# distributed-lab/era-boojum

Measured on AMD Instinct MI355X. Metric: LDE+Merkle commit Goldilocks elems/s (2^22x256, LDE x4), higher is better.
Workload: dtype u64 (Goldilocks); 1 GPU; C3: 2^22 rows x 256 cols, LDE x4, Poseidon2 cap 16; rows=4194304, cols=256, lde=4, cap=16, tree_hasher=poseidon2, parallelism=single, launch=stream

## Files before the change

### era-boojum_amd/csrc/gl_asm.hpp

```cpp
#pragma once
#include <stdint.h>

namespace glasm {

__device__ __forceinline__ void mul_x1(uint32_t a00, uint32_t a10, uint32_t b00, uint32_t b10, uint32_t& z00, uint32_t& z10) {
    uint64_t q40, q42, q44, q64;
    asm volatile(
        "v_mad_u64_u32 v[2:3], %[q64], %[a10], %[b00], 0\n"
        "v_mad_u64_u32 v[0:1], %[q64], %[a00], %[b00], 0\n"
        "v_mad_u64_u32 v[4:5], %[q44], %[a00], %[b10], v[2:3]\n"
        "v_mad_u64_u32 v[6:7], %[q64], %[a10], %[b10], 0\n"
        "v_add_co_u32 v1, %[q40], v1, v4\n"
        "v_addc_co_u32 v7, %[q64], v7, 0, %[q44]\n"
        "s_nop 0\n"
        "v_addc_co_u32 v5, %[q42], v5, v6, %[q40]\n"
        "s_nop 1\n"
        "v_subb_co_u32 v0, %[q40], v0, v7, %[q42]\n"
        "s_nop 1\n"
        "v_subb_co_u32 v1, %[q40], v1, 0, %[q40]\n"
        "s_nop 1\n"
        "v_subb_co_u32 v5, %[q40], v5, 0, %[q40]\n"
        "v_mad_u64_u32 v[2:3], %[q42], v5, -1, v[0:1]\n"
        "s_nop 1\n"
        "v_cndmask_b32_e64 v8, 0, -1, %[q42]\n"
// ... 72 lines not shown
        "v_addc_co_u32 v25, %[q54], v25, v26, %[q52]\n"
        "v_subb_co_u32 v0, %[q40], v0, v7, %[q42]\n"
        "v_subb_co_u32 v10, %[q46], v10, v17, %[q48]\n"
        "v_subb_co_u32 v20, %[q52], v20, v27, %[q54]\n"
        "v_subb_co_u32 v1, %[q40], v1, 0, %[q40]\n"
        "v_subb_co_u32 v11, %[q46], v11, 0, %[q46]\n"
        "v_subb_co_u32 v21, %[q52], v21, 0, %[q52]\n"
        "v_subb_co_u32 v5, %[q40], v5, 0, %[q40]\n"
        "v_subb_co_u32 v15, %[q46], v15, 0, %[q46]\n"
        "v_subb_co_u32 v25, %[q52], v25, 0, %[q52]\n"
        "v_mad_u64_u32 v[2:3], %[q42], v5, -1, v[0:1]\n"
        "v_mad_u64_u32 v[12:13], %[q48], v15, -1, v[10:11]\n"
        "v_mad_u64_u32 v[22:23], %[q54], v25, -1, v[20:21]\n"
        "v_cndmask_b32_e64 v8, 0, -1, %[q42]\n"
        "v_cndmask_b32_e64 v18, 0, -1, %[q48]\n"
        "v_cndmask_b32_e64 v28, 0, -1, %[q54]\n"
        "v_addc_co_u32 %[z00], %[q42], v2, v8, %[q40]\n"
        "v_addc_co_u32 %[z01], %[q48], v12, v18, %[q46]\n"
        "v_addc_co_u32 %[z02], %[q54], v22, v28, %[q52]\n"
        "v_addc_co_u32 %[z10], %[q64], v3, 0, %[q42]\n"
        "v_addc_co_u32 %[z11], %[q64], v13, 0, %[q48]\n"
        "v_addc_co_u32 %[z12], %[q64], v23, 0, %[q54]\n"
        : [z00] "=&v"(z00), [z10] "=&v"(z10), [z01] "=&v"(z01), [z11] "=&v"(z11), [z02] "=&v"(z02), [z12] "=&v"(z12), [q40] "=&s"(q40), [q42] "=&s"(q42), [q44] "=&s"(q44), [q46] "=&s"(q46), [q48] "=&s"(q48), [q50] "=&s"(q50), [q52] "=&s"(q52), [q54] "=&s"(q54), [q56] "=&s"(q56), [q64] "=&s"(q64)
        : [a00] "v"(a00), [a10] "v"(a10), [b00] "v"(b00), [b10] "v"(b10), [a01] "v"(a01), [a11] "v"(a11), [b01] "v"(b01), [b11] "v"(b11), [a02] "v"(a02), [a12] "v"(a12), [b02] "v"(b02), [b12] "v"(b12)
        : "v0", "v1", "v2", "v3", "v4", "v5", "v6", "v7", "v8", "v9", "v10", "v11", "v12", "v13", "v14", "v15", "v16", "v17", "v18", "v19", "v20", "v21", "v22", "v23", "v24", "v25", "v26", "v27", "v28", "v29");
}

__device__ __forceinline__ void mul_x4(uint32_t a00, uint32_t a10, uint32_t b00, uint32_t b10, uint32_t& z00, uint32_t& z10, uint32_t a01, uint32_t a11, uint32_t b01, uint32_t b11, uint32_t& z01, uint32_t& z11, uint32_t a02, uint32_t a12, uint32_t b02, uint32_t b12, uint32_t& z02, uint32_t& z12, uint32_t a03, uint32_t a13, uint32_t b03, uint32_t b13, uint32_t& z03, uint32_t& z13) {
    uint64_t q40, q42, q44, q46, q48, q50, q52, q54, q56, q58, q60, q62, q64;
    asm volatile(
        "v_mad_u64_u32 v[2:3], %[q64], %[a10], %[b00], 0\n"
        "v_mad_u64_u32 v[12:13], %[q64], %[a11], %[b01], 0\n"
        "v_mad_u64_u32 v[22:23], %[q64], %[a12], %[b02], 0\n"
        "v_mad_u64_u32 v[32:33], %[q64], %[a13], %[b03], 0\n"
        "v_mad_u64_u32 v[0:1], %[q64], %[a00], %[b00], 0\n"
        "v_mad_u64_u32 v[10:11], %[q64], %[a01], %[b01], 0\n"
        "v_mad_u64_u32 v[20:21], %[q64], %[a02], %[b02], 0\n"
        "v_mad_u64_u32 v[30:31], %[q64], %[a03], %[b03], 0\n"
        "v_mad_u64_u32 v[4:5], %[q44], %[a00], %[b10], v[2:3]\n"
        "v_mad_u64_u32 v[14:15], %[q50], %[a01], %[b11], v[12:13]\n"
        "v_mad_u64_u32 v[24:25], %[q56], %[a02], %[b12], v[22:23]\n"
        "v_mad_u64_u32 v[34:35], %[q62], %[a03], %[b13], v[32:33]\n"
        "v_mad_u64_u32 v[6:7], %[q64], %[a10], %[b10], 0\n"
        "v_mad_u64_u32 v[16:17], %[q64], %[a11], %[b11], 0\n"
        "v_mad_u64_u32 v[26:27], %[q64], %[a12], %[b12], 0\n"
        "v_mad_u64_u32 v[36:37], %[q64], %[a13], %[b13], 0\n"
        "v_add_co_u32 v1, %[q40], v1, v4\n"
        "v_add_co_u32 v11, %[q46], v11, v14\n"
        "v_add_co_u32 v21, %[q52], v21, v24\n"
        "v_add_co_u32 v31, %[q58], v31, v34\n"
        "v_addc_co_u32 v7, %[q64], v7, 0, %[q44]\n"
        "v_addc_co_u32 v17, %[q64], v17, 0, %[q50]\n"
        "v_addc_co_u32 v27, %[q64], v27, 0, %[q56]\n"
        "v_addc_co_u32 v37, %[q64], v37, 0, %[q62]\n"
        "v_addc_co_u32 v5, %[q42], v5, v6, %[q40]\n"
        "v_addc_co_u32 v15, %[q48], v15, v16, %[q46]\n"
        "v_addc_co_u32 v25, %[q54], v25, v26, %[q52]\n"
        "v_addc_co_u32 v35, %[q60], v35, v36, %[q58]\n"
        "v_subb_co_u32 v0, %[q40], v0, v7, %[q42]\n"
        "v_subb_co_u32 v10, %[q46], v10, v17, %[q48]\n"
        "v_subb_co_u32 v20, %[q52], v20, v27, %[q54]\n"
        "v_subb_co_u32 v30, %[q58], v30, v37, %[q60]\n"
        "v_subb_co_u32 v1, %[q40], v1, 0, %[q40]\n"
        "v_subb_co_u32 v11, %[q46], v11, 0, %[q46]\n"
        "v_subb_co_u32 v21, %[q52], v21, 0, %[q52]\n"
        "v_subb_co_u32 v31, %[q58], v31, 0, %[q58]\n"
        "v_subb_co_u32 v5, %[q40], v5, 0, %[q40]\n"
        "v_subb_co_u32 v15, %[q46], v15, 0, %[q46]\n"
        "v_subb_co_u32 v25, %[q52], v25, 0, %[q52]\n"
        "v_subb_co_u32 v35, %[q58], v35, 0, %[q58]\n"
        "v_mad_u64_u32 v[2:3], %[q42], v5, -1, v[0:1]\n"
        "v_mad_u64_u32 v[12:13], %[q48], v15, -1, v[10:11]\n"
        "v_mad_u64_u32 v[22:23], %[q54], v25, -1, v[20:21]\n"
        "v_mad_u64_u32 v[32:33], %[q60], v35, -1, v[30:31]\n"
        "v_cndmask_b32_e64 v8, 0, -1, %[q42]\n"
        "v_cndmask_b32_e64 v18, 0, -1, %[q48]\n"
        "v_cndmask_b32_e64 v28, 0, -1, %[q54]\n"
        "v_cndmask_b32_e64 v38, 0, -1, %[q60]\n"
        "v_addc_co_u32 %[z00], %[q42], v2, v8, %[q40]\n"
        "v_addc_co_u32 %[z01], %[q48], v12, v18, %[q46]\n"
        "v_addc_co_u32 %[z02], %[q54], v22, v28, %[q52]\n"
        "v_addc_co_u32 %[z03], %[q60], v32, v38, %[q58]\n"
        "v_addc_co_u32 %[z10], %[q64], v3, 0, %[q42]\n"
        "v_addc_co_u32 %[z11], %[q64], v13, 0, %[q48]\n"
        "v_addc_co_u32 %[z12], %[q64], v23, 0, %[q54]\n"
        "v_addc_co_u32 %[z13], %[q64], v33, 0, %[q60]\n"
        : [z00] "=&v"(z00), [z10] "=&v"(z10), [z01] "=&v"(z01), [z11] "=&v"(z11), [z02] "=&v"(z02), [z12] "=&v"(z12), [z03] "=&v"(z03), [z13] "=&v"(z13), [q40] "=&s"(q40), [q42] "=&s"(q42), [q44] "=&s"(q44), [q46] "=&s"(q46), [q48] "=&s"(q48), [q50] "=&s"(q50), [q52] "=&s"(q52), [q54] "=&s"(q54), [q56] "=&s"(q56), [q58] "=&s"(q58), [q60] "=&s"(q60), [q62] "=&s"(q62), [q64] "=&s"(q64)
        : [a00] "v"(a00), [a10] "v"(a10), [b00] "v"(b00), [b10] "v"(b10), [a01] "v"(a01), [a11] "v"(a11), [b01] "v"(b01), [b11] "v"(b11), [a02] "v"(a02), [a12] "v"(a12), [b02] "v"(b02), [b12] "v"(b12), [a03] "v"(a03), [a13] "v"(a13), [b03] "v"(b03), [b13] "v"(b13)
        : "v0", "v1", "v2", "v3", "v4", "v5", "v6", "v7", "v8", "v9", "v10", "v11", "v12", "v13", "v14", "v15", "v16", "v17", "v18", "v19", "v20", "v21", "v22", "v23", "v24", "v25", "v26", "v27", "v28", "v29", "v30", "v31", "v32", "v33", "v34", "v35", "v36", "v37", "v38", "v39");
}

__device__ __forceinline__ void mul_sb_x4(uint32_t a00, uint32_t a10, uint32_t b00, uint32_t b10, uint32_t& z00, uint32_t& z10, uint32_t a01, uint32_t a11, uint32_t b01, uint32_t b11, uint32_t& z01, uint32_t& z11, uint32_t a02, uint32_t a12, uint32_t b02, uint32_t b12, uint32_t& z02, uint32_t& z12, uint32_t a03, uint32_t a13, uint32_t b03, uint32_t b13, uint32_t& z03, uint32_t& z13) {
    uint64_t q40, q42, q44, q46, q48, q50, q52, q54, q56, q58, q60, q62, q64;
    asm volatile(
        "v_mad_u64_u32 v[2:3], %[q64], %[a10], %[b00], 0\n"
        "v_mad_u64_u32 v[12:13], %[q64], %[a11], %[b01], 0\n"
        "v_mad_u64_u32 v[22:23], %[q64], %[a12], %[b02], 0\n"
        "v_mad_u64_u32 v[32:33], %[q64], %[a13], %[b03], 0\n"
        "v_mad_u64_u32 v[0:1], %[q64], %[a00], %[b00], 0\n"
        "v_mad_u64_u32 v[10:11], %[q64], %[a01], %[b01], 0\n"
        "v_mad_u64_u32 v[20:21], %[q64], %[a02], %[b02], 0\n"
        "v_mad_u64_u32 v[30:31], %[q64], %[a03], %[b03], 0\n"
        "v_mad_u64_u32 v[4:5], %[q44], %[a00], %[b10], v[2:3]\n"
        "v_mad_u64_u32 v[14:15], %[q50], %[a01], %[b11], v[12:13]\n"
        "v_mad_u64_u32 v[24:25], %[q56], %[a02], %[b12], v[22:23]\n"
        "v_mad_u64_u32 v[34:35], %[q62], %[a03], %[b13], v[32:33]\n"
        "v_mad_u64_u32 v[6:7], %[q64], %[a10], %[b10], 0\n"
        "v_mad_u64_u32 v[16:17], %[q64], %[a11], %[b11], 0\n"
        "v_mad_u64_u32 v[26:27], %[q64], %[a12], %[b12], 0\n"
        "v_mad_u64_u32 v[36:37], %[q64], %[a13], %[b13], 0\n"
        "v_add_co_u32 v1, %[q40], v1, v4\n"
        "v_add_co_u32 v11, %[q46], v11, v14\n"
        "v_add_co_u32 v21, %[q52], v21, v24\n"
        "v_add_co_u32 v31, %[q58], v31, v34\n"
        "v_addc_co_u32 v7, %[q64], v7, 0, %[q44]\n"
        "v_addc_co_u32 v17, %[q64], v17, 0, %[q50]\n"
        "v_addc_co_u32 v27, %[q64], v27, 0, %[q56]\n"
        "v_addc_co_u32 v37, %[q64], v37, 0, %[q62]\n"
        "v_addc_co_u32 v5, %[q42], v5, v6, %[q40]\n"
        "v_addc_co_u32 v15, %[q48], v15, v16, %[q46]\n"
        "v_addc_co_u32 v25, %[q54], v25, v26, %[q52]\n"
        "v_addc_co_u32 v35, %[q60], v35, v36, %[q58]\n"
        "v_subb_co_u32 v0, %[q40], v0, v7, %[q42]\n"
        "v_subb_co_u32 v10, %[q46], v10, v17, %[q48]\n"
        "v_subb_co_u32 v20, %[q52], v20, v27, %[q54]\n"
        "v_subb_co_u32 v30, %[q58], v30, v37, %[q60]\n"
        "v_subb_co_u32 v1, %[q40], v1, 0, %[q40]\n"
        "v_subb_co_u32 v11, %[q46], v11, 0, %[q46]\n"
        "v_subb_co_u32 v21, %[q52], v21, 0, %[q52]\n"
        "v_subb_co_u32 v31, %[q58], v31, 0, %[q58]\n"
        "v_subb_co_u32 v5, %[q40], v5, 0, %[q40]\n"
        "v_subb_co_u32 v15, %[q46], v15, 0, %[q46]\n"
        "v_subb_co_u32 v25, %[q52], v25, 0, %[q52]\n"
        "v_subb_co_u32 v35, %[q58], v35, 0, %[q58]\n"
        "v_mad_u64_u32 v[2:3], %[q42], v5, -1, v[0:1]\n"
        "v_mad_u64_u32 v[12:13], %[q48], v15, -1, v[10:11]\n"
        "v_mad_u64_u32 v[22:23], %[q54], v25, -1, v[20:21]\n"
        "v_mad_u64_u32 v[32:33], %[q60], v35, -1, v[30:31]\n"
        "v_cndmask_b32_e64 v8, 0, -1, %[q42]\n"
        "v_cndmask_b32_e64 v18, 0, -1, %[q48]\n"
        "v_cndmask_b32_e64 v28, 0, -1, %[q54]\n"
        "v_cndmask_b32_e64 v38, 0, -1, %[q60]\n"
        "v_addc_co_u32 %[z00], %[q42], v2, v8, %[q40]\n"
        "v_addc_co_u32 %[z01], %[q48], v12, v18, %[q46]\n"
        "v_addc_co_u32 %[z02], %[q54], v22, v28, %[q52]\n"
        "v_addc_co_u32 %[z03], %[q60], v32, v38, %[q58]\n"
        "v_addc_co_u32 %[z10], %[q64], v3, 0, %[q42]\n"
        "v_addc_co_u32 %[z11], %[q64], v13, 0, %[q48]\n"
        "v_addc_co_u32 %[z12], %[q64], v23, 0, %[q54]\n"
        "v_addc_co_u32 %[z13], %[q64], v33, 0, %[q60]\n"
        : [z00] "=&v"(z00), [z10] "=&v"(z10), [z01] "=&v"(z01), [z11] "=&v"(z11), [z02] "=&v"(z02), [z12] "=&v"(z12), [z03] "=&v"(z03), [z13] "=&v"(z13), [q40] "=&s"(q40), [q42] "=&s"(q42), [q44] "=&s"(q44), [q46] "=&s"(q46), [q48] "=&s"(q48), [q50] "=&s"(q50), [q52] "=&s"(q52), [q54] "=&s"(q54), [q56] "=&s"(q56), [q58] "=&s"(q58), [q60] "=&s"(q60), [q62] "=&s"(q62), [q64] "=&s"(q64)
        : [a00] "v"(a00), [a10] "v"(a10), [b00] "s"(b00), [b10] "s"(b10), [a01] "v"(a01), [a11] "v"(a11), [b01] "s"(b01), [b11] "s"(b11), [a02] "v"(a02), [a12] "v"(a12), [b02] "s"(b02), [b12] "s"(b12), [a03] "v"(a03), [a13] "v"(a13), [b03] "s"(b03), [b13] "s"(b13)
        : "v0", "v1", "v2", "v3", "v4", "v5", "v6", "v7", "v8", "v9", "v10", "v11", "v12", "v13", "v14", "v15", "v16", "v17", "v18", "v19", "v20", "v21", "v22", "v23", "v24", "v25", "v26", "v27", "v28", "v29", "v30", "v31", "v32", "v33", "v34", "v35", "v36", "v37", "v38", "v39");
}

__device__ __forceinline__ void reduce_x1(uint64_t L0, uint32_t Hlo0, uint32_t Hhi0, uint64_t& z0) {
    uint64_t q40, q64;
    asm volatile(
        "v_mad_u64_u32 v[0:1], %[q64], %[Hhi0], -1, %[L0]\n"
        "v_add_co_u32 v1, %[q40], v1, %[Hlo0]\n"
        "s_nop 1\n"
        "v_cndmask_b32_e64 v2, 0, -1, %[q40]\n"
        "v_mad_u64_u32 %[z0], %[q64], v2, 1, v[0:1]\n"
        : [z0] "=&v"(z0), [q40] "=&s"(q40), [q64] "=&s"(q64)
        : [L0] "v"(L0), [Hlo0] "v"(Hlo0), [Hhi0] "v"(Hhi0)
        : "v0", "v1", "v2", "v3");
}

__device__ __forceinline__ void reduce_x2(uint64_t L0, uint32_t Hlo0, uint32_t Hhi0, uint64_t& z0, uint64_t L1, uint32_t Hlo1, uint32_t Hhi1, uint64_t& z1) {
    uint64_t q40, q44, q64;
    asm volatile(
        "v_mad_u64_u32 v[0:1], %[q64], %[Hhi0], -1, %[L0]\n"
        "v_mad_u64_u32 v[4:5], %[q64], %[Hhi1], -1, %[L1]\n"
        "v_add_co_u32 v1, %[q40], v1, %[Hlo0]\n"
        "v_add_co_u32 v5, %[q44], v5, %[Hlo1]\n"
        "s_nop 0\n"
        "v_cndmask_b32_e64 v2, 0, -1, %[q40]\n"
        "v_cndmask_b32_e64 v6, 0, -1, %[q44]\n"
        "v_mad_u64_u32 %[z0], %[q64], v2, 1, v[0:1]\n"
        "v_mad_u64_u32 %[z1], %[q64], v6, 1, v[4:5]\n"
        : [z0] "=&v"(z0), [z1] "=&v"(z1), [q40] "=&s"(q40), [q44] "=&s"(q44), [q64] "=&s"(q64)
        : [L0] "v"(L0), [Hlo0] "v"(Hlo0), [Hhi0] "v"(Hhi0), [L1] "v"(L1), [Hlo1] "v"(Hlo1), [Hhi1] "v"(Hhi1)
        : "v0", "v1", "v2", "v3", "v4", "v5", "v6", "v7");
}

__device__ __forceinline__ void reduce_x3(uint64_t L0, uint32_t Hlo0, uint32_t Hhi0, uint64_t& z0, uint64_t L1, uint32_t Hlo1, uint32_t Hhi1, uint64_t& z1, uint64_t L2, uint32_t Hlo2, uint32_t Hhi2, uint64_t& z2) {
    uint64_t q40, q44, q48, q64;
    asm volatile(
        "v_mad_u64_u32 v[0:1], %[q64], %[Hhi0], -1, %[L0]\n"
        "v_mad_u64_u32 v[4:5], %[q64], %[Hhi1], -1, %[L1]\n"
        "v_mad_u64_u32 v[8:9], %[q64], %[Hhi2], -1, %[L2]\n"
        "v_add_co_u32 v1, %[q40], v1, %[Hlo0]\n"
        "v_add_co_u32 v5, %[q44], v5, %[Hlo1]\n"
        "v_add_co_u32 v9, %[q48], v9, %[Hlo2]\n"
        "v_cndmask_b32_e64 v2, 0, -1, %[q40]\n"
        "v_cndmask_b32_e64 v6, 0, -1, %[q44]\n"
        "v_cndmask_b32_e64 v10, 0, -1, %[q48]\n"
        "v_mad_u64_u32 %[z0], %[q64], v2, 1, v[0:1]\n"
        "v_mad_u64_u32 %[z1], %[q64], v6, 1, v[4:5]\n"
        "v_mad_u64_u32 %[z2], %[q64], v10, 1, v[8:9]\n"
        : [z0] "=&v"(z0), [z1] "=&v"(z1), [z2] "=&v"(z2), [q40] "=&s"(q40), [q44] "=&s"(q44), [q48] "=&s"(q48), [q64] "=&s"(q64)
        : [L0] "v"(L0), [Hlo0] "v"(Hlo0), [Hhi0] "v"(Hhi0), [L1] "v"(L1), [Hlo1] "v"(Hlo1), [Hhi1] "v"(Hhi1), [L2] "v"(L2), [Hlo2] "v"(Hlo2), [Hhi2] "v"(Hhi2)
        : "v0", "v1", "v2", "v3", "v4", "v5", "v6", "v7", "v8", "v9", "v10", "v11");
}

__device__ __forceinline__ void reduce_x4(uint64_t L0, uint32_t Hlo0, uint32_t Hhi0, uint64_t& z0, uint64_t L1, uint32_t Hlo1, uint32_t Hhi1, uint64_t& z1, uint64_t L2, uint32_t Hlo2, uint32_t Hhi2, uint64_t& z2, uint64_t L3, uint32_t Hlo3, uint32_t Hhi3, uint64_t& z3) {
    uint64_t q40, q44, q48, q52, q64;
    asm volatile(
        "v_mad_u64_u32 v[0:1], %[q64], %[Hhi0], -1, %[L0]\n"
        "v_mad_u64_u32 v[4:5], %[q64], %[Hhi1], -1, %[L1]\n"
        "v_mad_u64_u32 v[8:9], %[q64], %[Hhi2], -1, %[L2]\n"
        "v_mad_u64_u32 v[12:13], %[q64], %[Hhi3], -1, %[L3]\n"
        "v_add_co_u32 v1, %[q40], v1, %[Hlo0]\n"
        "v_add_co_u32 v5, %[q44], v5, %[Hlo1]\n"
        "v_add_co_u32 v9, %[q48], v9, %[Hlo2]\n"
        "v_add_co_u32 v13, %[q52], v13, %[Hlo3]\n"
        "v_cndmask_b32_e64 v2, 0, -1, %[q40]\n"
        "v_cndmask_b32_e64 v6, 0, -1, %[q44]\n"
        "v_cndmask_b32_e64 v10, 0, -1, %[q48]\n"
        "v_cndmask_b32_e64 v14, 0, -1, %[q52]\n"
        "v_mad_u64_u32 %[z0], %[q64], v2, 1, v[0:1]\n"
        "v_mad_u64_u32 %[z1], %[q64], v6, 1, v[4:5]\n"
        "v_mad_u64_u32 %[z2], %[q64], v10, 1, v[8:9]\n"
        "v_mad_u64_u32 %[z3], %[q64], v14, 1, v[12:13]\n"
        : [z0] "=&v"(z0), [z1] "=&v"(z1), [z2] "=&v"(z2), [z3] "=&v"(z3), [q40] "=&s"(q40), [q44] "=&s"(q44), [q48] "=&s"(q48), [q52] "=&s"(q52), [q64] "=&s"(q64)
        : [L0] "v"(L0), [Hlo0] "v"(Hlo0), [Hhi0] "v"(Hhi0), [L1] "v"(L1), [Hlo1] "v"(Hlo1), [Hhi1] "v"(Hhi1), [L2] "v"(L2), [Hlo2] "v"(Hlo2), [Hhi2] "v"(Hhi2), [L3] "v"(L3), [Hlo3] "v"(Hlo3), [Hhi3] "v"(Hhi3)
        : "v0", "v1", "v2", "v3", "v4", "v5", "v6", "v7", "v8", "v9", "v10", "v11", "v12", "v13", "v14", "v15");
}

__device__ __forceinline__ void add_x1(uint32_t a00, uint32_t a10, uint32_t b00, uint32_t b10, uint32_t& z00, uint32_t& z10) {
    uint64_t q40;
    asm volatile(
        "v_add_co_u32 %[z00], %[q40], %[a00], %[b00]\n"
        "s_nop 1\n"
        "v_addc_co_u32 %[z10], %[q40], %[a10], %[b10], %[q40]\n"
        "s_nop 1\n"
        "v_cndmask_b32_e64 v0, 0, -1, %[q40]\n"
        "v_add_co_u32 %[z00], %[q40], %[z00], v0\n"
        "s_nop 1\n"
        "v_addc_co_u32 %[z10], %[q40], %[z10], 0, %[q40]\n"
        "s_nop 1\n"
        "v_cndmask_b32_e64 v0, 0, -1, %[q40]\n"
        "v_add_co_u32 %[z00], %[q40], %[z00], v0\n"
        "s_nop 1\n"
        "v_addc_co_u32 %[z10], %[q40], %[z10], 0, %[q40]\n"
        : [z00] "=&v"(z00), [z10] "=&v"(z10), [q40] "=&s"(q40)
        : [a00] "v"(a00), [a10] "v"(a10), [b00] "v"(b00), [b10] "v"(b10)
        : "v0", "v1");
}

__device__ __forceinline__ void sub_x1(uint32_t a00, uint32_t a10, uint32_t b00, uint32_t b10, uint32_t& z00, uint32_t& z10) {
    uint64_t q40;
    asm volatile(
        "v_sub_co_u32 %[z00], %[q40], %[a00], %[b00]\n"
        "s_nop 1\n"
        "v_subb_co_u32 %[z10], %[q40], %[a10], %[b10], %[q40]\n"
        "s_nop 1\n"
        "v_cndmask_b32_e64 v0, 0, -1, %[q40]\n"
        "v_sub_co_u32 %[z00], %[q40], %[z00], v0\n"
        "s_nop 1\n"
        "v_subb_co_u32 %[z10], %[q40], %[z10], 0, %[q40]\n"
        "s_nop 1\n"
        "v_cndmask_b32_e64 v0, 0, -1, %[q40]\n"
        "v_sub_co_u32 %[z00], %[q40], %[z00], v0\n"
        "s_nop 1\n"
        "v_subb_co_u32 %[z10], %[q40], %[z10], 0, %[q40]\n"
        : [z00] "=&v"(z00), [z10] "=&v"(z10), [q40] "=&s"(q40)
        : [a00] "v"(a00), [a10] "v"(a10), [b00] "v"(b00), [b10] "v"(b10)
        : "v0", "v1");
}

__device__ __forceinline__ void add_x2(uint32_t a00, uint32_t a10, uint32_t b00, uint32_t b10, uint32_t& z00, uint32_t& z10, uint32_t a01, uint32_t a11, uint32_t b01, uint32_t b11, uint32_t& z01, uint32_t& z11) {
    uint64_t q40, q44;
    asm volatile(
        "v_add_co_u32 %[z00], %[q40], %[a00], %[b00]\n"
        "v_add_co_u32 %[z01], %[q44], %[a01], %[b01]\n"
        "s_nop 0\n"
        "v_addc_co_u32 %[z10], %[q40], %[a10], %[b10], %[q40]\n"
        "v_addc_co_u32 %[z11], %[q44], %[a11], %[b11], %[q44]\n"
        "s_nop 0\n"
        "v_cndmask_b32_e64 v0, 0, -1, %[q40]\n"
        "v_cndmask_b32_e64 v2, 0, -1, %[q44]\n"
        "v_add_co_u32 %[z00], %[q40], %[z00], v0\n"
        "v_add_co_u32 %[z01], %[q44], %[z01], v2\n"
        "s_nop 0\n"
        "v_addc_co_u32 %[z10], %[q40], %[z10], 0, %[q40]\n"
        "v_addc_co_u32 %[z11], %[q44], %[z11], 0, %[q44]\n"
        "s_nop 0\n"
        "v_cndmask_b32_e64 v0, 0, -1, %[q40]\n"
        "v_cndmask_b32_e64 v2, 0, -1, %[q44]\n"
        "v_add_co_u32 %[z00], %[q40], %[z00], v0\n"
        "v_add_co_u32 %[z01], %[q44], %[z01], v2\n"
        "s_nop 0\n"
        "v_addc_co_u32 %[z10], %[q40], %[z10], 0, %[q40]\n"
        "v_addc_co_u32 %[z11], %[q44], %[z11], 0, %[q44]\n"
        : [z00] "=&v"(z00), [z10] "=&v"(z10), [z01] "=&v"(z01), [z11] "=&v"(z11), [q40] "=&s"(q40), [q44] "=&s"(q44)
        : [a00] "v"(a00), [a10] "v"(a10), [b00] "v"(b00), [b10] "v"(b10), [a01] "v"(a01), [a11] "v"(a11), [b01] "v"(b01), [b11] "v"(b11)
        : "v0", "v1", "v2", "v3");
}

__device__ __forceinline__ void sub_x2(uint32_t a00, uint32_t a10, uint32_t b00, uint32_t b10, uint32_t& z00, uint32_t& z10, uint32_t a01, uint32_t a11, uint32_t b01, uint32_t b11, uint32_t& z01, uint32_t& z11) {
    uint64_t q40, q44;
    asm volatile(
        "v_sub_co_u32 %[z00], %[q40], %[a00], %[b00]\n"
        "v_sub_co_u32 %[z01], %[q44], %[a01], %[b01]\n"
        "s_nop 0\n"
// ... 791 lines not shown
```

### era-boojum_amd/csrc/poseidon2.hpp

```cpp
#pragma once
#include "gl.hpp"
#include "gl_asm.hpp"

namespace p2 {

struct RcLimbs {
    uint64_t lo[30][12];
    uint64_t hi[30][12];
};

constexpr uint64_t RC_FLAT[30][12] = {
#include "poseidon2_rc.inc"
};

constexpr RcLimbs make_rc_limbs() {
    RcLimbs r{};
    for (int i = 0; i < 30; i++)
        for (int j = 0; j < 12; j++) {
            r.lo[i][j] = RC_FLAT[i][j] & 0xFFFFFFFFull;
            r.hi[i][j] = RC_FLAT[i][j] >> 32;
        }
    return r;
}

__device__ __constant__ static const RcLimbs RCL = make_rc_limbs();

namespace sched {
constexpr uint64_t P = 0xFFFFFFFF00000001ull;
constexpr uint64_t addm(uint64_t a, uint64_t b) { return (uint64_t)(((unsigned __int128)a + b) % P); }
constexpr uint64_t subm(uint64_t a, uint64_t b) { return addm(a, P - b % P); }
constexpr uint64_t mulm(uint64_t a, uint64_t b) { return (uint64_t)(((unsigned __int128)a * b) % P); }
constexpr int SH[12] = {4, 14, 11, 8, 0, 5, 2, 9, 13, 6, 3, 12};
constexpr uint64_t FULL_RC_BOUND = ~0ull - (1ull << 41) + 1;
constexpr uint64_t LIMB_RC_BOUND = (1ull << 63) + (1ull << 62);
struct Values {
    uint64_t k[11];
    uint64_t d[10];
    uint64_t rc26[12];
};
constexpr Values derive() {
    Values v{};
    uint64_t f[12] = {RC_FLAT[4][0]};
    for (int q = 0; q < 11; q++) {
        const int r = 4 + 2 * q;
        uint64_t s = 0;
        for (int i = 1; i < 12; i++) s = addm(s, f[i]);
        v.k[q] = subm(RC_FLAT[r + 1][0], s);
        f[0] = 0;
        for (int i = 0; i < 12; i++) f[i] = addm(addm(mulm(f[i], 1ull << SH[i]), s), v.k[q]);
        s = 0;
        for (int i = 1; i < 12; i++) s = addm(s, f[i]);
        f[0] = 0;
        for (int i = 0; i < 12; i++) f[i] = addm(mulm(f[i], 1ull << SH[i]), s);
        if (q < 10) {
            v.d[q] = subm(RC_FLAT[r + 2][0], f[0]);
            f[0] = RC_FLAT[r + 2][0];
        }
    }
    for (int i = 0; i < 12; i++) v.rc26[i] = subm(RC_FLAT[26][i], f[i]);
    return v;
}
constexpr Values V = derive();
constexpr bool full_rcs_fit() {
    for (int r : {0, 1, 2, 3, 27, 28, 29})
        for (int i = 0; i < 12; i++)
            if (RC_FLAT[r][i] >= FULL_RC_BOUND) return false;
    return RC_FLAT[4][0] < FULL_RC_BOUND;
}
static_assert(full_rcs_fit(), "a full-round constant is too large for the one-add form");
}

struct Sched {
    uint64_t rcw8[30][8];
    uint64_t rcw4[30][4];
    uint64_t k_lo[11], k_hi[11];
    uint64_t d_lo[10], d_hi[10];
    uint64_t rc26_w[12], rc26_lo[12], rc26_hi[12];
};
constexpr Sched make_sched() {
    Sched s{};
    for (int r = 0; r < 30; r++)
        for (int i = 0; i < 12; i++) (i < 8 ? s.rcw8[r][i] : s.rcw4[r][i - 8]) = RC_FLAT[r][i];
    for (int q = 0; q < 11; q++) { s.k_lo[q] = sched::V.k[q] & 0xFFFFFFFFull; s.k_hi[q] = sched::V.k[q] >> 32; }
    for (int q = 0; q < 10; q++) { s.d_lo[q] = sched::V.d[q] & 0xFFFFFFFFull; s.d_hi[q] = sched::V.d[q] >> 32; }
    for (int i = 0; i < 12; i++) {
        s.rc26_w[i] = sched::V.rc26[i];
        s.rc26_lo[i] = sched::V.rc26[i] & 0xFFFFFFFFull;
        s.rc26_hi[i] = sched::V.rc26[i] >> 32;
    }
    return s;
}
__device__ __constant__ static const Sched SCH = make_sched();

struct State {
    uint32_t lo[12], hi[12];
};

__device__ __forceinline__ void sbox_x4(uint32_t* lo, uint32_t* hi) {
    uint32_t a0, a1, b0, b1, c0, c1, d0, d1;
    glasm::mul_x4(lo[0], hi[0], lo[0], hi[0], a0, a1, lo[1], hi[1], lo[1], hi[1], b0, b1,
                  lo[2], hi[2], lo[2], hi[2], c0, c1, lo[3], hi[3], lo[3], hi[3], d0, d1);
    uint32_t e0, e1, f0, f1, g0, g1, h0, h1;
    glasm::mul_x4(a0, a1, lo[0], hi[0], e0, e1, b0, b1, lo[1], hi[1], f0, f1,
                  c0, c1, lo[2], hi[2], g0, g1, d0, d1, lo[3], hi[3], h0, h1);
    uint32_t i0, i1, j0, j1, k0, k1, l0, l1;
    glasm::mul_x4(a0, a1, a0, a1, i0, i1, b0, b1, b0, b1, j0, j1,
                  c0, c1, c0, c1, k0, k1, d0, d1, d0, d1, l0, l1);
    glasm::mul_x4(e0, e1, i0, i1, lo[0], hi[0], f0, f1, j0, j1, lo[1], hi[1],
                  g0, g1, k0, k1, lo[2], hi[2], h0, h1, l0, l1, lo[3], hi[3]);
}

__device__ __forceinline__ void sbox_x1(uint32_t& lo, uint32_t& hi) {
    uint32_t a0, a1, e0, e1, i0, i1;
    glasm::mul_x1(lo, hi, lo, hi, a0, a1);
    glasm::mul_x2(a0, a1, lo, hi, e0, e1, a0, a1, a0, a1, i0, i1);
    glasm::mul_x1(e0, e1, i0, i1, lo, hi);
}

__device__ __forceinline__ void m4_limbs(uint64_t& x0, uint64_t& x1, uint64_t& x2, uint64_t& x3) {
    uint64_t t0 = x0 + x1;
    uint64_t t1 = x2 + x3;
    uint64_t t2 = (x1 << 1) + t1;
    uint64_t t3 = (x3 << 1) + t0;
    uint64_t t4 = (t1 << 2) + t3;
    uint64_t t5 = (t0 << 2) + t2;
    uint64_t t6 = t3 + t5;
    uint64_t t7 = t2 + t4;
    x0 = t6; x1 = t5; x2 = t7; x3 = t4;
}

__device__ __forceinline__ uint64_t add_lo_u64(uint32_t lo, uint64_t b) {
    uint64_t r;
    asm volatile("v_mad_u64_u32 %0, vcc, %1, 1, %2" : "=v"(r) : "v"(lo), "s"(b) : "vcc");
    return r;
}

enum Out { OUT_ALL = 0, OUT_CAP = 1, OUT_DIGEST = 2 };

template <int OUT = OUT_ALL>
__device__ __forceinline__ void mds_ext_limbs(const uint32_t* v, uint64_t* X) {
#pragma unroll
    for (int i = 0; i < 12; i++) X[i] = v[i];
    m4_limbs(X[0], X[1], X[2], X[3]);
    m4_limbs(X[4], X[5], X[6], X[7]);
    m4_limbs(X[8], X[9], X[10], X[11]);
#pragma unroll
    for (int i = 0; i < 4; i++) {
        uint64_t a = X[i], b = X[i + 4], c = X[i + 8];
        if constexpr (OUT == OUT_ALL) {
            uint64_t s = a + b + c;
            X[i] = s + a;
            X[i + 4] = s + b;
            X[i + 8] = s + c;
        } else if constexpr (OUT == OUT_CAP) {
            X[i + 8] = (c << 1) + a + b;
        } else {
            X[i] = (a << 1) + b + c;
        }
    }
}

__device__ __forceinline__ void split(uint64_t z, uint32_t& lo, uint32_t& hi) {
    lo = (uint32_t)z;
    hi = (uint32_t)(z >> 32);
}

template <int OUT = OUT_ALL>
__device__ __forceinline__ void reduce12(const uint64_t* L, const uint64_t* H, uint32_t* lo, uint32_t* hi) {
#pragma unroll
    for (int q = 0; q < 3; q++) {
        if constexpr (OUT == OUT_CAP) { if (q != 2) continue; }
        if constexpr (OUT == OUT_DIGEST) { if (q != 0) continue; }
        const int i = 4 * q;
        uint64_t z[4];
        glasm::reduce_x4(L[i], (uint32_t)H[i], (uint32_t)(H[i] >> 32), z[0],
                         L[i + 1], (uint32_t)H[i + 1], (uint32_t)(H[i + 1] >> 32), z[1],
                         L[i + 2], (uint32_t)H[i + 2], (uint32_t)(H[i + 2] >> 32), z[2],
                         L[i + 3], (uint32_t)H[i + 3], (uint32_t)(H[i + 3] >> 32), z[3]);
#pragma unroll
        for (int j = 0; j < 4; j++) split(z[j], lo[i + j], hi[i + j]);
    }
}

template <int OUT = OUT_ALL, bool RC = true>
__device__ __forceinline__ void full_round(State& s, uint64_t* L, uint64_t* H, int r) {
    if constexpr (RC) {
#pragma unroll
        for (int i = 0; i < 12; i++) L[i] += i < 8 ? SCH.rcw8[r][i] : SCH.rcw4[r][i - 8];
    }
    reduce12(L, H, s.lo, s.hi);
#pragma unroll
    for (int q = 0; q < 3; q++) sbox_x4(s.lo + 4 * q, s.hi + 4 * q);
    mds_ext_limbs<OUT>(s.lo, L);
    mds_ext_limbs<OUT>(s.hi, H);
}

struct Partial {
    uint64_t z0;
    uint64_t W[12];
    uint32_t G[12];
};

template <bool HALF>
__device__ __forceinline__ void partial_first(const Partial& P, int q, uint64_t* L, uint64_t* H, uint32_t& lo0,
                                              uint32_t& hi0) {
    uint64_t z0;
    uint32_t lo[12], hi[12];
    const uint64_t kl = SCH.k_lo[q], kh = SCH.k_hi[q];
    split(P.z0, lo[0], hi[0]);
#pragma unroll
    for (int i = 1; i < 12; i++) split(P.W[i], lo[i], hi[i]);
    sbox_x1(lo[0], hi[0]);
    if constexpr (HALF) glasm::mi_layer_a_g(lo, hi, P.G, kl, kh, L, H, z0);
    else glasm::mi_layer_a(lo, hi, kl, kh, L, H, z0);
    split(z0, lo0, hi0);
    sbox_x1(lo0, hi0);
}

template <bool HALF>
__device__ __forceinline__ void partial_round_pair(Partial& P, int q) {
    uint64_t L[12], H[12], Lo[12], Ho[12];
    uint32_t lo0, hi0, hh[12];
    const uint64_t dl = SCH.d_lo[q], dh = SCH.d_hi[q];
    partial_first<HALF>(P, q, L, H, lo0, hi0);
    glasm::mi_layer_b_half(lo0, hi0, L, H, dl, dh, Lo, Ho, P.z0);
#pragma unroll
    for (int i = 1; i < 12; i++) split(Ho[i], P.G[i], hh[i]);
    glasm::eps_fold_x11(hh, Lo, P.W);
}

__device__ __forceinline__ void partial_round_pair_last(const Partial& P, uint64_t* Lo, uint64_t* Ho) {
    uint64_t L[12], H[12];
    uint32_t lo0, hi0;
    partial_first<true>(P, 10, L, H, lo0, hi0);
    glasm::mi_layer_b_limbs(lo0, hi0, L, H, Lo, Ho);
}

template <int I = 0>
__device__ __forceinline__ void add_rc26(uint64_t* L, uint64_t* H) {
    if constexpr (sched::V.rc26[I] < sched::LIMB_RC_BOUND) {
        L[I] += SCH.rc26_w[I];
    } else {
        L[I] += SCH.rc26_lo[I];
        H[I] += SCH.rc26_hi[I];
    }
    if constexpr (I + 1 < 12) add_rc26<I + 1>(L, H);
}

template <int OUT = OUT_ALL>
__device__ __forceinline__ void permute(State& s) {
    uint64_t L[12], H[12], Z[12];
    Partial P;
    mds_ext_limbs(s.lo, L);
    mds_ext_limbs(s.hi, H);
#pragma unroll 1
    for (int r = 0; r < 4; r++) full_round(s, L, H, r);
    L[0] += SCH.rcw8[4][0];
#pragma unroll
    for (int q = 0; q < 3; q++) {
        const int i = 4 * q;
        glasm::reduce_x4(L[i], (uint32_t)H[i], (uint32_t)(H[i] >> 32), Z[i],
                         L[i + 1], (uint32_t)H[i + 1], (uint32_t)(H[i + 1] >> 32), Z[i + 1],
                         L[i + 2], (uint32_t)H[i + 2], (uint32_t)(H[i + 2] >> 32), Z[i + 2],
                         L[i + 3], (uint32_t)H[i + 3], (uint32_t)(H[i + 3] >> 32), Z[i + 3]);
    }
    P.z0 = Z[0];
#pragma unroll
    for (int i = 1; i < 12; i++) P.W[i] = Z[i];
    partial_round_pair<false>(P, 0);
#pragma unroll 1
    for (int q = 1; q < 10; q++) partial_round_pair<true>(P, q);
    partial_round_pair_last(P, L, H);
    add_rc26(L, H);
    full_round<OUT_ALL, false>(s, L, H, 26);
#pragma unroll 1
    for (int r = 27; r < 29; r++) full_round(s, L, H, r);
    full_round<OUT>(s, L, H, 29);
    reduce12<OUT>(L, H, s.lo, s.hi);
}

__device__ __forceinline__ void permute(uint64_t v[12]) {
    State s;
#pragma unroll
    for (int i = 0; i < 12; i++) {
        s.lo[i] = (uint32_t)v[i];
        s.hi[i] = (uint32_t)(v[i] >> 32);
    }
    permute(s);
#pragma unroll
    for (int i = 0; i < 12; i++) v[i] = ((uint64_t)s.hi[i] << 32) | s.lo[i];
}

}
```

Baseline: 5.826 billion elems/s.

## Fuse last S-box multiply with lazy unreduced output feeding the MDS

```diff
diff --git a/era-boojum_amd/csrc/gl_asm.hpp b/era-boojum_amd/csrc/gl_asm.hpp
--- a/era-boojum_amd/csrc/gl_asm.hpp
+++ b/era-boojum_amd/csrc/gl_asm.hpp
@@ -248,6 +248,64 @@
         : [z00] "=&v"(z00), [z10] "=&v"(z10), [z01] "=&v"(z01), [z11] "=&v"(z11), [z02] "=&v"(z02), [z12] "=&v"(z12), [z03] "=&v"(z03), [z13] "=&v"(z13), [q40] "=&s"(q40), [q42] "=&s"(q42), [q44] "=&s"(q44), [q46] "=&s"(q46), [q48] "=&s"(q48), [q50] "=&s"(q50), [q52] "=&s"(q52), [q54] "=&s"(q54), [q56] "=&s"(q56), [q58] "=&s"(q58), [q60] "=&s"(q60), [q62] "=&s"(q62), [q64] "=&s"(q64)
         : [a00] "v"(a00), [a10] "v"(a10), [b00] "s"(b00), [b10] "s"(b10), [a01] "v"(a01), [a11] "v"(a11), [b01] "s"(b01), [b11] "s"(b11), [a02] "v"(a02), [a12] "v"(a12), [b02] "s"(b02), [b12] "s"(b12), [a03] "v"(a03), [a13] "v"(a13), [b03] "s"(b03), [b13] "s"(b13)
         : "v0", "v1", "v2", "v3", "v4", "v5", "v6", "v7", "v8", "v9", "v10", "v11", "v12", "v13", "v14", "v15", "v16", "v17", "v18", "v19", "v20", "v21", "v22", "v23", "v24", "v25", "v26", "v27", "v28", "v29", "v30", "v31", "v32", "v33", "v34", "v35", "v36", "v37", "v38", "v39");
+}
+
+__device__ __forceinline__ void mul_lazy_x4(uint32_t a00, uint32_t a10, uint32_t b00, uint32_t b10, uint64_t& Lin0, uint64_t& Hin0, uint32_t a01, uint32_t a11, uint32_t b01, uint32_t b11, uint64_t& Lin1, uint64_t& Hin1, uint32_t a02, uint32_t a12, uint32_t b02, uint32_t b12, uint64_t& Lin2, uint64_t& Hin2, uint32_t a03, uint32_t a13, uint32_t b03, uint32_t b13, uint64_t& Lin3, uint64_t& Hin3) {
+    uint64_t q40, q42, q44, q46, q48, q50, q52, q54, q56, q58, q60, q62, q64;
+    asm volatile(
+        "v_mov_b32 v33, 0\n"
+        "v_mov_b32 v35, 0\n"
+        "v_mad_u64_u32 v[2:3], %[q64], %[a10], %[b00], 0\n"
+        "v_mad_u64_u32 v[10:11], %[q64], %[a11], %[b01], 0\n"
+        "v_mad_u64_u32 v[18:19], %[q64], %[a12], %[b02], 0\n"
+        "v_mad_u64_u32 v[26:27], %[q64], %[a13], %[b03], 0\n"
+        "v_mad_u64_u32 v[0:1], %[q64], %[a00], %[b00], 0\n"
+        "v_mad_u64_u32 v[8:9], %[q64], %[a01], %[b01], 0\n"
+        "v_mad_u64_u32 v[16:17], %[q64], %[a02], %[b02], 0\n"
+        "v_mad_u64_u32 v[24:25], %[q64], %[a03], %[b03], 0\n"
+        "v_mad_u64_u32 v[4:5], %[q44], %[a00], %[b10], v[2:3]\n"
+        "v_mad_u64_u32 v[12:13], %[q50], %[a01], %[b11], v[10:11]\n"
+        "v_mad_u64_u32 v[20:21], %[q56], %[a02], %[b12], v[18:19]\n"
+        "v_mad_u64_u32 v[28:29], %[q62], %[a03], %[b13], v[26:27]\n"
+        "v_mad_u64_u32 v[6:7], %[q64], %[a10], %[b10], 0\n"
+        "v_mad_u64_u32 v[14:15], %[q64], %[a11], %[b11], 0\n"
+        "v_mad_u64_u32 v[22:23], %[q64], %[a12], %[b12], 0\n"
+        "v_mad_u64_u32 v[30:31], %[q64], %[a13], %[b13], 0\n"
+        "v_add_co_u32 v1, %[q40], v1, v4\n"
+        "v_add_co_u32 v9, %[q46], v9, v12\n"
+        "v_add_co_u32 v17, %[q52], v17, v20\n"
+        "v_add_co_u32 v25, %[q58], v25, v28\n"
+        "v_addc_co_u32 v7, %[q64], v7, 0, %[q44]\n"
+        "v_addc_co_u32 v15, %[q64], v15, 0, %[q50]\n"
+        "v_addc_co_u32 v23, %[q64], v23, 0, %[q56]\n"
+        "v_addc_co_u32 v31, %[q64], v31, 0, %[q62]\n"
+        "v_addc_co_u32 v32, %[q42], v5, v6, %[q40]\n"
+        "v_addc_co_u32 v34, %[q48], v13, v14, %[q46]\n"
+        "v_mad_u64_u32 %[Hin0], %[q64], v1, 1, v[32:33]\n"
+        "v_mad_u64_u32 %[Hin1], %[q64], v9, 1, v[34:35]\n"
+        "v_not_b32 v32, v32\n"
+        "v_not_b32 v34, v34\n"
+        "v_subb_co_u32 v2, %[q64], -1, v7, %[q42]\n"
+        "v_subb_co_u32 v10, %[q64], -1, v15, %[q48]\n"
+        "v_mad_u64_u32 %[Lin0], %[q64], v0, 1, v[32:33]\n"
+        "v_mad_u64_u32 %[Lin1], %[q64], v8, 1, v[34:35]\n"
+        "v_mad_u64_u32 %[Lin0], %[q64], v2, 1, %[Lin0]\n"
+        "v_mad_u64_u32 %[Lin1], %[q64], v10, 1, %[Lin1]\n"
+        "v_addc_co_u32 v32, %[q54], v21, v22, %[q52]\n"
+        "v_addc_co_u32 v34, %[q60], v29, v30, %[q58]\n"
+        "v_mad_u64_u32 %[Hin2], %[q64], v17, 1, v[32:33]\n"
+        "v_mad_u64_u32 %[Hin3], %[q64], v25, 1, v[34:35]\n"
+        "v_not_b32 v32, v32\n"
+        "v_not_b32 v34, v34\n"
+        "v_subb_co_u32 v18, %[q64], -1, v23, %[q54]\n"
+        "v_subb_co_u32 v26, %[q64], -1, v31, %[q60]\n"
+        "v_mad_u64_u32 %[Lin2], %[q64], v16, 1, v[32:33]\n"
+        "v_mad_u64_u32 %[Lin3], %[q64], v24, 1, v[34:35]\n"
+        "v_mad_u64_u32 %[Lin2], %[q64], v18, 1, %[Lin2]\n"
+        "v_mad_u64_u32 %[Lin3], %[q64], v26, 1, %[Lin3]\n"
+        : [Lin0] "=&v"(Lin0), [Hin0] "=&v"(Hin0), [Lin1] "=&v"(Lin1), [Hin1] "=&v"(Hin1), [Lin2] "=&v"(Lin2), [Hin2] "=&v"(Hin2), [Lin3] "=&v"(Lin3), [Hin3] "=&v"(Hin3), [q40] "=&s"(q40), [q42] "=&s"(q42), [q44] "=&s"(q44), [q46] "=&s"(q46), [q48] "=&s"(q48), [q50] "=&s"(q50), [q52] "=&s"(q52), [q54] "=&s"(q54), [q56] "=&s"(q56), [q58] "=&s"(q58), [q60] "=&s"(q60), [q62] "=&s"(q62), [q64] "=&s"(q64)
+        : [a00] "v"(a00), [a10] "v"(a10), [b00] "v"(b00), [b10] "v"(b10), [a01] "v"(a01), [a11] "v"(a11), [b01] "v"(b01), [b11] "v"(b11), [a02] "v"(a02), [a12] "v"(a12), [b02] "v"(b02), [b12] "v"(b12), [a03] "v"(a03), [a13] "v"(a13), [b03] "v"(b03), [b13] "v"(b13)
+        : "v0", "v1", "v2", "v3", "v4", "v5", "v6", "v7", "v8", "v9", "v10", "v11", "v12", "v13", "v14", "v15", "v16", "v17", "v18", "v19", "v20", "v21", "v22", "v23", "v24", "v25", "v26", "v27", "v28", "v29", "v30", "v31", "v32", "v33", "v34", "v35");
 }
 
 __device__ __forceinline__ void reduce_x1(uint64_t L0, uint32_t Hlo0, uint32_t Hhi0, uint64_t& z0) {
diff --git a/era-boojum_amd/csrc/poseidon2.hpp b/era-boojum_amd/csrc/poseidon2.hpp
--- a/era-boojum_amd/csrc/poseidon2.hpp
+++ b/era-boojum_amd/csrc/poseidon2.hpp
@@ -68,6 +68,25 @@
     return RC_FLAT[4][0] < FULL_RC_BOUND;
 }
 static_assert(full_rcs_fit(), "a full-round constant is too large for the one-add form");
+
+constexpr uint64_t LAZY_OFF = 2 * 0xFFFFFFFFull;
+constexpr uint64_t me_row_sum(int i) { return (i & 1) ? 48 : 64; }
+constexpr uint64_t lazy_off(int i) { return me_row_sum(i) * LAZY_OFF; }
+constexpr uint64_t lazy_fix_lo(int i) { return 1 + 2 * me_row_sum(i); }
+constexpr uint64_t lazy_fix_hi(int i) { return 0xFFFFFFFFull - 2 * me_row_sum(i); }
+constexpr bool lazy_in(int r) { return (r >= 1 && r <= 3) || (r >= 27 && r <= 29); }
+constexpr bool lazy_rcs_fit() {
+    for (int r = 0; r < 30; r++)
+        for (int i = 0; i < 12; i++)
+            if ((lazy_in(r) || (r == 4 && i == 0)) &&
+                (RC_FLAT[r][i] < lazy_off(i) || RC_FLAT[r][i] - lazy_off(i) >= FULL_RC_BOUND))
+                return false;
+    return true;
+}
+static_assert(lazy_rcs_fit(), "a full-round constant is smaller than the lazy offset it takes out");
+static_assert((lazy_fix_lo(0) + (lazy_fix_hi(0) << 32) + lazy_off(0)) == P &&
+                  (lazy_fix_lo(1) + (lazy_fix_hi(1) << 32) + lazy_off(1)) == P,
+              "the two-limb form of -lazy_off");
 }
 
 struct Sched {
@@ -76,11 +95,17 @@
     uint64_t k_lo[11], k_hi[11];
     uint64_t d_lo[10], d_hi[10];
     uint64_t rc26_w[12], rc26_lo[12], rc26_hi[12];
+    uint64_t rcl8[30][8];
+    uint64_t rcl4[30][4];
 };
 constexpr Sched make_sched() {
     Sched s{};
     for (int r = 0; r < 30; r++)
-        for (int i = 0; i < 12; i++) (i < 8 ? s.rcw8[r][i] : s.rcw4[r][i - 8]) = RC_FLAT[r][i];
+        for (int i = 0; i < 12; i++) {
+            (i < 8 ? s.rcw8[r][i] : s.rcw4[r][i - 8]) = RC_FLAT[r][i];
+            const bool lazy = sched::lazy_in(r) || (r == 4 && i == 0);
+            (i < 8 ? s.rcl8[r][i] : s.rcl4[r][i - 8]) = RC_FLAT[r][i] - (lazy ? sched::lazy_off(i) : 0);
+        }
     for (int q = 0; q < 11; q++) { s.k_lo[q] = sched::V.k[q] & 0xFFFFFFFFull; s.k_hi[q] = sched::V.k[q] >> 32; }
     for (int q = 0; q < 10; q++) { s.d_lo[q] = sched::V.d[q] & 0xFFFFFFFFull; s.d_hi[q] = sched::V.d[q] >> 32; }
     for (int i = 0; i < 12; i++) {
@@ -96,7 +121,7 @@
     uint32_t lo[12], hi[12];
 };
 
-__device__ __forceinline__ void sbox_x4(uint32_t* lo, uint32_t* hi) {
+__device__ __forceinline__ void sbox_lazy_x4(const uint32_t* lo, const uint32_t* hi, uint64_t* Lin, uint64_t* Hin) {
     uint32_t a0, a1, b0, b1, c0, c1, d0, d1;
     glasm::mul_x4(lo[0], hi[0], lo[0], hi[0], a0, a1, lo[1], hi[1], lo[1], hi[1], b0, b1,
                   lo[2], hi[2], lo[2], hi[2], c0, c1, lo[3], hi[3], lo[3], hi[3], d0, d1);
@@ -106,8 +131,8 @@
     uint32_t i0, i1, j0, j1, k0, k1, l0, l1;
     glasm::mul_x4(a0, a1, a0, a1, i0, i1, b0, b1, b0, b1, j0, j1,
                   c0, c1, c0, c1, k0, k1, d0, d1, d0, d1, l0, l1);
-    glasm::mul_x4(e0, e1, i0, i1, lo[0], hi[0], f0, f1, j0, j1, lo[1], hi[1],
-                  g0, g1, k0, k1, lo[2], hi[2], h0, h1, l0, l1, lo[3], hi[3]);
+    glasm::mul_lazy_x4(e0, e1, i0, i1, Lin[0], Hin[0], f0, f1, j0, j1, Lin[1], Hin[1],
+                       g0, g1, k0, k1, Lin[2], Hin[2], h0, h1, l0, l1, Lin[3], Hin[3]);
 }
 
 __device__ __forceinline__ void sbox_x1(uint32_t& lo, uint32_t& hi) {
@@ -138,9 +163,7 @@
 enum Out { OUT_ALL = 0, OUT_CAP = 1, OUT_DIGEST = 2 };
 
 template <int OUT = OUT_ALL>
-__device__ __forceinline__ void mds_ext_limbs(const uint32_t* v, uint64_t* X) {
-#pragma unroll
-    for (int i = 0; i < 12; i++) X[i] = v[i];
+__device__ __forceinline__ void mds_ext_limbs(uint64_t* X) {
     m4_limbs(X[0], X[1], X[2], X[3]);
     m4_limbs(X[4], X[5], X[6], X[7]);
     m4_limbs(X[8], X[9], X[10], X[11]);
@@ -160,6 +183,13 @@
     }
 }
 
+template <int OUT = OUT_ALL>
+__device__ __forceinline__ void mds_ext_limbs(const uint32_t* v, uint64_t* X) {
+#pragma unroll
+    for (int i = 0; i < 12; i++) X[i] = v[i];
+    mds_ext_limbs<OUT>(X);
+}
+
 __device__ __forceinline__ void split(uint64_t z, uint32_t& lo, uint32_t& hi) {
     lo = (uint32_t)z;
     hi = (uint32_t)(z >> 32);
@@ -186,13 +216,24 @@
 __device__ __forceinline__ void full_round(State& s, uint64_t* L, uint64_t* H, int r) {
     if constexpr (RC) {
 #pragma unroll
-        for (int i = 0; i < 12; i++) L[i] += i < 8 ? SCH.rcw8[r][i] : SCH.rcw4[r][i - 8];
+        for (int i = 0; i < 12; i++) L[i] += i < 8 ? SCH.rcl8[r][i] : SCH.rcl4[r][i - 8];
     }
     reduce12(L, H, s.lo, s.hi);
 #pragma unroll
-    for (int q = 0; q < 3; q++) sbox_x4(s.lo + 4 * q, s.hi + 4 * q);
-    mds_ext_limbs<OUT>(s.lo, L);
-    mds_ext_limbs<OUT>(s.hi, H);
+    for (int q = 0; q < 3; q++) sbox_lazy_x4(s.lo + 4 * q, s.hi + 4 * q, L + 4 * q, H + 4 * q);
+    mds_ext_limbs<OUT>(L);
+    mds_ext_limbs<OUT>(H);
+}
+
+template <int I>
+__device__ __forceinline__ void lazy_fix(uint64_t* L, uint64_t* H) {
+    L[I] += sched::lazy_fix_lo(I);
+    H[I] += sched::lazy_fix_hi(I);
+}
+template <int I, int N>
+__device__ __forceinline__ void lazy_fix_range(uint64_t* L, uint64_t* H) {
+    lazy_fix<I>(L, H);
+    if constexpr (I + 1 < N) lazy_fix_range<I + 1, N>(L, H);
 }
 
 struct Partial {
@@ -255,7 +296,8 @@
     mds_ext_limbs(s.hi, H);
 #pragma unroll 1
     for (int r = 0; r < 4; r++) full_round(s, L, H, r);
-    L[0] += SCH.rcw8[4][0];
+    L[0] += SCH.rcl8[4][0];
+    lazy_fix_range<1, 12>(L, H);
 #pragma unroll
     for (int q = 0; q < 3; q++) {
         const int i = 4 * q;
@@ -276,6 +318,9 @@
 #pragma unroll 1
     for (int r = 27; r < 29; r++) full_round(s, L, H, r);
     full_round<OUT>(s, L, H, 29);
+    if constexpr (OUT == OUT_ALL) lazy_fix_range<0, 12>(L, H);
+    else if constexpr (OUT == OUT_CAP) lazy_fix_range<8, 12>(L, H);
+    else lazy_fix_range<0, 4>(L, H);
     reduce12<OUT>(L, H, s.lo, s.hi);
 }
 
```

New measurement: 5.911 billion elems/s, median of 6. 1.01x the previous value.
